# kdexd/probnmn-clevr

Hardware: AMD Instinct MI355X
Metric: CLEVR questions/sec (joint_training step) (higher is better)
Workload: dtype f32; 1 GPU; joint_training_ours.yml (NMN + seq2seq + REINFORCE), global batch 1024 = 1024 questions per GPU x 1 (BASELINE configs[3]), 14x14x1024 features, half of the batch with program supervision, fwd+bwd+[all-reduce]+clamp+Adam; global_batch=1024, per_gpu_batch=1024, parallelism=dp1

## Files before the change

### probnmn-clevr_amd/csrc/gemm.hip

```cpp
#include <hip/hip_runtime.h>
#include <stdint.h>

#include <type_traits>

#include "../../include/probnmn_hip.h"
#include "global_ptr.h"
#include "lds_optin.h"

namespace {

typedef float f32x16 __attribute__((ext_vector_type(16)));
using pnmn::as_global;
using pnmn::gfloat;

constexpr int TM = 128, TN = 128, TK = 32;
constexpr int OP_FLOATS = TM * TK;
using lchar = __attribute__((address_space(3))) char;
using gchar = __attribute__((address_space(1))) char;

struct Batch {
    pnmn_gemm_desc d[PNMN_GEMM_MAX];
    int first[PNMN_GEMM_MAX + 1];
    int n;
};

template <bool KC>
__device__ __forceinline__ void load_tile(const gfloat* base, int64_t ld, int row0, int k0, int rows, int K, bool vec, int tid,
                                          f32x4 (&r)[4], int shift_t, const gfloat* h0, int64_t ld_h0) {
#pragma unroll
    for (int j = 0; j < 4; ++j) {
        const int p = tid + 256 * j;
        f32x4 v = f32x4{0.f, 0.f, 0.f, 0.f};
        if (KC) {
            const int row = row0 + (p >> 3), k = k0 + 4 * (p & 7);
            if (row < rows && k < K) {
                const gfloat* src = base + (int64_t)row * ld + k;
                if (vec && k + 3 < K) {
                    v = pnmn::load4(src);
                } else {
#pragma unroll
                    for (int e = 0; e < 4; ++e)
                        if (k + e < K) v[e] = src[e];
                }
            }
        } else {
            const int k = k0 + (p >> 5), row = row0 + 4 * (p & 31);
            if (k < K && row < rows) {
                const gfloat* src;
                bool zero = false;
                if (shift_t > 0) {
                    const int b = k / shift_t;
                    if (k - b * shift_t == 0) {
                        zero = h0 == nullptr;
                        src = h0 + (int64_t)b * ld_h0 + row;
                    } else {
                        src = base + (int64_t)(k - 1) * ld + row;
                    }
                } else {
                    src = base + (int64_t)k * ld + row;
                }
                if (!zero) {
                    if (vec && row + 3 < rows) {
                        v = pnmn::load4(src);
                    } else {
#pragma unroll
                        for (int e = 0; e < 4; ++e)
                            if (row + e < rows) v[e] = src[e];
                    }
                }
            }
        }
        r[j] = v;
    }
}

__device__ __forceinline__ void load_tile_shift(const gfloat* base, int64_t ld, int col0, int k0, int tid, f32x4 (&r)[4], int shift_t,
                                                float rcp_t, const gfloat* h0, int64_t ld_h0) {
#pragma unroll
    for (int j = 0; j < 4; ++j) {
        const int k = k0 + (tid >> 5) + 8 * j, col = col0 + 4 * (tid & 31);
        const int b = (int)(((float)k + 0.5f) * rcp_t);
        const bool first = k == b * shift_t;
        const gfloat* prev = base + (int64_t)(k - 1) * ld + col;
        const gfloat* init = h0 ? h0 + (int64_t)b * ld_h0 + col : base + col;
        f32x4 v = pnmn::load4(first ? init : prev);
        if (first && !h0) v = f32x4{0.f, 0.f, 0.f, 0.f};
        r[j] = v;
    }
}

template <bool KC>
__device__ __forceinline__ void store_tile(float* lds, int tid, const f32x4 (&r)[4]) {
#pragma unroll
    for (int j = 0; j < 4; ++j) {
        const int p = tid + 256 * j;
        if (KC) {
            const int row = p >> 3;
            *reinterpret_cast<f32x4*>(lds + row * TK + 4 * ((p & 7) ^ ((row >> 1) & 7))) = r[j];
        } else {
            *reinterpret_cast<f32x4*>(lds + (p >> 5) * TM + 4 * (p & 31)) = r[j];
        }
    }
}

template <bool KC>
__device__ __forceinline__ f32x4 frag(const float* lds, int row, int q, int h) {
    if (KC) return *reinterpret_cast<const f32x4*>(lds + row * TK + 4 * ((2 * q + h) ^ ((row >> 1) & 7)));
    const float* p = lds + (8 * q + 4 * h) * TM + row;
    return f32x4{p[0], p[TM], p[2 * TM], p[3 * TM]};
}

template <bool KC>
struct Direct {
    const gchar* base;
    uint32_t v0, v1;
    int64_t piece, step;
    uint32_t off;

    __device__ __forceinline__ void start(const gfloat* origin, int64_t ld, int row0, int k0, int tid) {
        const int wave = __builtin_amdgcn_readfirstlane(tid >> 6), lane = tid & 63;
        const uint64_t o64 = (uint64_t)(uintptr_t)origin;
        const gchar* o = (const gchar*)(((uint64_t)(uint32_t)__builtin_amdgcn_readfirstlane((int)(o64 >> 32)) << 32) |
                                        (uint32_t)__builtin_amdgcn_readfirstlane((int)(uint32_t)o64));
        if (KC) {
            const int c = (lane & 7) ^ (lane >> 4);
            base = o + ((int64_t)(row0 + 32 * wave) * ld + k0) * 4;
            v0 = (uint32_t)((lane >> 3) * ld) * 4u + 16u * c, v1 = (uint32_t)((lane >> 3) * ld) * 4u + 16u * (c ^ 4);
            piece = 32 * ld, step = 4 * TK, off = (uint32_t)wave * 32u * 128u;
        } else {
            base = o + ((int64_t)(k0 + 8 * wave) * ld + row0) * 4;
            v0 = v1 = (uint32_t)((lane >> 5) * ld) * 4u + 16u * (lane & 31);
            piece = 8 * ld, step = 4 * (int64_t)TK * ld, off = (uint32_t)wave * 8u * 512u;
        }
    }
    __device__ __forceinline__ void issue(float* tile) {
        const uint32_t dst = __builtin_amdgcn_readfirstlane((uint32_t)(uintptr_t)((lchar*)tile)) + off;
#pragma unroll
        for (int j = 0; j < 4; ++j) {
            const uint64_t src = (uint64_t)(uintptr_t)(base + j * piece);
            asm volatile("s_mov_b32 m0, %2\n\ts_nop 0\n\tglobal_load_lds_dwordx4 %0, %1"
                         :
                         : "v"(KC && (j & 1) ? v1 : v0), "s"(src), "s"(dst + 1024u * j)
                         : "memory");
        }
        base += step;
    }
};

template <bool AKC, bool BKC>
__device__ __forceinline__ void mac_tile(const float* ca, const float* cb, int wm, int wn, int i, int h, f32x16 (&acc)[2][2], bool want_cs,
                                         float (&cs)[2]) {
#pragma unroll
    for (int q = 0; q < 4; ++q) {
        f32x4 a[2], b[2];
#pragma unroll
        for (int t = 0; t < 2; ++t) {
            a[t] = frag<AKC>(ca, 64 * wm + 32 * t + i, q, h);
            b[t] = frag<BKC>(cb, 64 * wn + 32 * t + i, q, h);
        }
        if (!AKC && want_cs) {
#pragma unroll
            for (int t = 0; t < 2; ++t) cs[t] += (a[t][0] + a[t][1]) + (a[t][2] + a[t][3]);
        }
#pragma unroll
        for (int s = 0; s < 4; ++s)
#pragma unroll
            for (int mt = 0; mt < 2; ++mt)
#pragma unroll
                for (int nt = 0; nt < 2; ++nt)
                    acc[mt][nt] = __builtin_amdgcn_mfma_f32_32x32x2f32(a[mt][s], b[nt][s], acc[mt][nt], 0, 0, 0);
    }
}

template <bool AKC, bool BKC>
__device__ __forceinline__ void contract(const pnmn_gemm_desc& d, int m0, int n0, int kbeg, int kend, float* lds, f32x16 (&acc)[2][2],
                                         bool want_cs, float (&cs)[2]) {
    const int tid = threadIdx.x, wave = tid >> 6, lane = tid & 63, i = lane & 31, h = lane >> 5;
    const int wm = wave >> 1, wn = wave & 1;
    const gfloat* A = as_global(d.a);
    const gfloat* Bm = as_global(d.b);
    const gfloat* h0 = as_global(d.shift_h0);
    const bool avec = (d.lda & 3) == 0 && ((uintptr_t)d.a & 15) == 0;
    const bool bvec = (d.ldb & 3) == 0 && ((uintptr_t)d.b & 15) == 0 && (d.shift_t == 0 || d.shift_h0 == nullptr ||
                                                                       ((d.ld_h0 & 3) == 0 && ((uintptr_t)d.shift_h0 & 15) == 0));
    float* la = lds;
    float* lb = lds + 2 * OP_FLOATS;
    const bool adir = avec && m0 + TM <= d.M, bdir = bvec && n0 + TN <= d.N && (BKC || d.shift_t == 0);
    const int kfull = kbeg + (kend - kbeg) / TK * TK;
    const float rcp_t = d.shift_t > 0 ? 1.f / (float)d.shift_t : 0.f;
    Direct<AKC> da;
    Direct<BKC> db;
    da.start(A, d.lda, m0, kbeg, tid);
    db.start(Bm, d.ldb, n0, kbeg, tid);
    auto loop = [&](auto ad_tag, auto bd_tag, int lo, int hi) {
        constexpr bool AD = decltype(ad_tag)::value, BD = decltype(bd_tag)::value;
        f32x4 ra[4], rb[4];
        auto fetch = [&](int k0, int st) {
            if constexpr (AD)
                da.issue(la + st * OP_FLOATS);
            else
                load_tile<AKC>(A, d.lda, m0, k0, d.M, kend, avec, tid, ra, 0, nullptr, 0);
            if constexpr (BD)
                db.issue(lb + st * OP_FLOATS);
            else if constexpr (AD && !BKC)
                load_tile_shift(Bm, d.ldb, n0, k0, tid, rb, d.shift_t, rcp_t, h0, d.ld_h0);
            else
                load_tile<BKC>(Bm, d.ldb, n0, k0, d.N, kend, bvec, tid, rb, BKC ? 0 : d.shift_t, h0, d.ld_h0);
        };
        auto commit = [&](int st) {
            if constexpr (!AD) store_tile<AKC>(la + st * OP_FLOATS, tid, ra);
            if constexpr (!BD) store_tile<BKC>(lb + st * OP_FLOATS, tid, rb);
        };
        if (lo >= hi) return;
        fetch(lo, 0);
        commit(0);
        asm volatile("s_waitcnt vmcnt(0)" ::: "memory");
        __syncthreads();
        int cur = 0;
        for (int k0 = lo; k0 < hi; k0 += TK) {
            const bool more = k0 + TK < hi;
            if (more) fetch(k0 + TK, cur ^ 1);
            const float* ca = la + cur * OP_FLOATS;
            const float* cb = lb + cur * OP_FLOATS;
            mac_tile<AKC, BKC>(ca, cb, wm, wn, i, h, acc, want_cs, cs);
            if (more) commit(cur ^ 1);
            asm volatile("s_waitcnt vmcnt(0)" ::: "memory");
            __syncthreads();
            cur ^= 1;
        }
    };
    using yes = std::true_type;
    using no = std::false_type;
    if (adir && bdir) {
        loop(yes{}, yes{}, kbeg, kfull);
        loop(no{}, no{}, kfull, kend);
    } else if (!BKC && adir && bvec && d.shift_t > 0 && n0 + TN <= d.N && kend <= (1 << 21)) {
        if constexpr (!BKC) {
            loop(yes{}, no{}, kbeg, kfull);
            loop(no{}, no{}, kfull, kend);
        }
    } else {
        loop(no{}, no{}, kbeg, kend);
    }
}

using gint2 = __attribute__((address_space(1))) int2;

__device__ __forceinline__ void load_rows(const gint2* list, int k0, int kend, int tid, int2 (&e)[4]) {
#pragma unroll
    for (int j = 0; j < 4; ++j) {
        const int k = k0 + (tid >> 5) + 8 * j;
        const gint2* q = list + (k < kend ? k : kend - 1);
        e[j].x = q->x, e[j].y = q->y;
    }
}

__device__ __forceinline__ void load_tile_rows(const gfloat* base, int64_t ld, int col0, int k0, int cols, int kend, bool vec, int tid,
                                               const int2 (&e)[4], f32x4 (&r)[4], bool shifted, const gfloat* h0, int64_t ld_h0) {
#pragma unroll
    for (int j = 0; j < 4; ++j) {
        const int k = k0 + (tid >> 5) + 8 * j, col = col0 + 4 * (tid & 31);
        f32x4 v = f32x4{0.f, 0.f, 0.f, 0.f};
        if (k < kend && col < cols) {
            const int row = shifted ? e[j].y : e[j].x;
            const bool first = row < 0;
            const gfloat* src = first ? (h0 ? h0 + (int64_t)(~row) * ld_h0 + col : base + col) : base + (int64_t)row * ld + col;
            if (vec && col + 3 < cols) {
                v = pnmn::load4(src);
            } else {
#pragma unroll
                for (int c = 0; c < 4; ++c)
                    if (col + c < cols) v[c] = src[c];
            }
            if (first && !h0) v = f32x4{0.f, 0.f, 0.f, 0.f};
        }
        r[j] = v;
    }
}

struct DirectRows {
    const gchar* origin;
    int64_t ld;
    uint32_t lane, off;

    __device__ __forceinline__ void start(const gfloat* base, int64_t ld_floats, int col0, int tid) {
        origin = (const gchar*)(base + col0), ld = 4 * ld_floats;
        lane = 16u * (tid & 31), off = (uint32_t)__builtin_amdgcn_readfirstlane(tid >> 6) * 1024u;
    }
    __device__ __forceinline__ void issue(float* tile, const int2 (&e)[4]) {
        const uint32_t dst = __builtin_amdgcn_readfirstlane((uint32_t)(uintptr_t)((lchar*)tile)) + off;
#pragma unroll
        for (int j = 0; j < 4; ++j) {
            const gchar* src = origin + (int64_t)e[j].x * ld + lane;
            asm volatile("s_mov_b32 m0, %1\n\ts_nop 0\n\tglobal_load_lds_dwordx4 %0, off" : : "v"(src), "s"(dst + 4096u * j) : "memory");
        }
    }
};

__device__ __forceinline__ void contract_rows(const pnmn_gemm_desc& d, const gint2* list, int m0, int n0, int kbeg, int kend, float* lds,
                                              f32x16 (&acc)[2][2], bool want_cs, float (&cs)[2]) {
    const int tid = threadIdx.x, wave = tid >> 6, lane = tid & 63, i = lane & 31, h = lane >> 5;
    const int wm = wave >> 1, wn = wave & 1;
    const gfloat* A = as_global(d.a);
    const gfloat* Bm = as_global(d.b);
    const gfloat* h0 = as_global(d.shift_h0);
    const bool shifted = d.shift_t > 0;
    const bool avec = (d.lda & 3) == 0 && ((uintptr_t)d.a & 15) == 0;
    const bool bvec = (d.ldb & 3) == 0 && ((uintptr_t)d.b & 15) == 0 &&
                      (!shifted || d.shift_h0 == nullptr || ((d.ld_h0 & 3) == 0 && ((uintptr_t)d.shift_h0 & 15) == 0));
    float* la = lds;
    float* lb = lds + 2 * OP_FLOATS;
    const bool adir = avec && m0 + TM <= d.M, bdir = bvec && n0 + TN <= d.N && !shifted;
    const int kfull = kbeg + (kend - kbeg) / TK * TK;
    DirectRows da, db;
    da.start(A, d.lda, m0, tid);
    db.start(Bm, d.ldb, n0, tid);
    auto loop = [&](auto ad_tag, auto bd_tag, int lo, int hi) {
        constexpr bool AD = decltype(ad_tag)::value, BD = decltype(bd_tag)::value;
        f32x4 ra[4], rb[4];
        int2 e[4];
        auto fetch = [&](int k0, int st) {
            if constexpr (AD)
                da.issue(la + st * OP_FLOATS, e);
            else
                load_tile_rows(A, d.lda, m0, k0, d.M, kend, avec, tid, e, ra, false, nullptr, 0);
            if constexpr (BD)
                db.issue(lb + st * OP_FLOATS, e);
            else
                load_tile_rows(Bm, d.ldb, n0, k0, d.N, kend, bvec, tid, e, rb, shifted, h0, d.ld_h0);
        };
        auto commit = [&](int st) {
            if constexpr (!AD) store_tile<false>(la + st * OP_FLOATS, tid, ra);
            if constexpr (!BD) store_tile<false>(lb + st * OP_FLOATS, tid, rb);
        };
        if (lo >= hi) return;
        load_rows(list, lo, kend, tid, e);
        fetch(lo, 0);
        load_rows(list, lo + TK, kend, tid, e);
        commit(0);
        asm volatile("s_waitcnt vmcnt(0)" ::: "memory");
        __syncthreads();
        int cur = 0;
        for (int k0 = lo; k0 < hi; k0 += TK) {
            const bool more = k0 + TK < hi;
            if (more) {
                fetch(k0 + TK, cur ^ 1);
                load_rows(list, k0 + 2 * TK, kend, tid, e);
            }
            mac_tile<false, false>(la + cur * OP_FLOATS, lb + cur * OP_FLOATS, wm, wn, i, h, acc, want_cs, cs);
            if (more) commit(cur ^ 1);
            asm volatile("s_waitcnt vmcnt(0)" ::: "memory");
            __syncthreads();
            cur ^= 1;
        }
    };
    using yes = std::true_type;
    using no = std::false_type;
    if (adir && bdir) {
        loop(yes{}, yes{}, kbeg, kfull);
        loop(no{}, no{}, kfull, kend);
    } else if (adir) {
        loop(yes{}, no{}, kbeg, kfull);
        loop(no{}, no{}, kfull, kend);
    } else {
        loop(no{}, no{}, kbeg, kend);
    }
}

struct Lists {
    const int2* rows[PNMN_GEMM_MAX];
    const int32_t* count[PNMN_GEMM_MAX];
};

template <bool LIST>
__global__ __launch_bounds__(256) __attribute__((amdgpu_waves_per_eu(2, 2))) void gemm_kernel(const Batch batch, const Lists lists) {
    extern __shared__ __attribute__((aligned(16))) float lds[];
    for (int unit = blockIdx.x; unit < batch.first[batch.n]; unit += gridDim.x) {
    int pi = 0;
    while (pi + 1 < batch.n && unit >= batch.first[pi + 1]) ++pi;
    const pnmn_gemm_desc d = batch.d[pi];
    const int local = unit - batch.first[pi];
    const int tiles_n = (d.N + TN - 1) / TN, tiles_m = (d.M + TM - 1) / TM;
    const int split = d.split_k > 1 ? d.split_k : 1;
    const int chunk = local % split, tile = local / split;
    const int tm = tile / tiles_n, tn = tile % tiles_n;
    const int m0 = tm * TM, n0 = tn * TN;
    int K = d.K;
    const gint2* list = nullptr;
    if constexpr (LIST) {
        list = (const gint2*)lists.rows[pi];
        if (list) {
            const int count = __builtin_amdgcn_readfirstlane(*(const __attribute__((address_space(1))) int32_t*)lists.count[pi]);
            K = count < 0 ? 0 : (count < d.K ? count : d.K);
        }
    }
    const int ktiles = (K + TK - 1) / TK;
    const int per = ktiles / split, extra = ktiles % split;
    const int kt0 = chunk * per + (chunk < extra ? chunk : extra);
    const int kt1 = kt0 + per + (chunk < extra ? 1 : 0);
    const int kbeg = kt0 * TK, kend = kt1 * TK < K ? kt1 * TK : K;

    f32x16 acc[2][2];
#pragma unroll
    for (int mt = 0; mt < 2; ++mt)
#pragma unroll
        for (int nt = 0; nt < 2; ++nt)
#pragma unroll
            for (int r = 0; r < 16; ++r) acc[mt][nt][r] = 0.f;
    const bool akc = !(d.flags & PNMN_GEMM_A_TRANSPOSED), bkc = (d.flags & PNMN_GEMM_B_TRANSPOSED) != 0;
    const bool want_cs = d.colsum != nullptr && !akc && tn == 0 && ((threadIdx.x >> 6) & 1) == 0;
    const bool tile_cs = d.colsum != nullptr && !akc && tn == 0;
    float cs[2] = {0.f, 0.f};
    if (LIST && list) {
        if (kbeg < kend) contract_rows(d, list, m0, n0, kbeg, kend, lds, acc, want_cs, cs);
    } else if (kbeg < kend) {
        if (akc && bkc)
            contract<true, true>(d, m0, n0, kbeg, kend, lds, acc, false, cs);
        else if (akc)
            contract<true, false>(d, m0, n0, kbeg, kend, lds, acc, false, cs);
        else if (bkc)
            contract<false, true>(d, m0, n0, kbeg, kend, lds, acc, want_cs, cs);
        else
            contract<false, false>(d, m0, n0, kbeg, kend, lds, acc, want_cs, cs);
    }

    int tid = threadIdx.x, m0e = m0, n0e = n0;
    asm volatile("" : "+v"(tid), "+s"(m0e), "+s"(n0e));
    const int wave = tid >> 6, lane = tid & 63, i = lane & 31, h = lane >> 5;
    const int wm = wave >> 1, wn = wave & 1;
    if (tile_cs) {
        if (want_cs) {
#pragma unroll
            for (int t = 0; t < 2; ++t) lds[h * TM + 64 * wm + 32 * t + i] = cs[t];
        }
        __syncthreads();
        if (tid < TM) {
            const float t = lds[tid] + lds[TM + tid];
            if (split > 1) {
                as_global(d.workspace)[(size_t)tiles_m * tiles_n * split * (TM * TN) + ((size_t)tm * split + chunk) * TM + tid] = t;
            } else if (m0e + tid < d.M) {
                d.colsum[m0e + tid] = t;
                if (d.colsum2) d.colsum2[m0e + tid] = t;
            }
        }
        __syncthreads();
    }
    if (split > 1) {
        gfloat* ws = as_global(d.workspace) + ((size_t)tile * split + chunk) * (TM * TN);
#pragma unroll
        for (int mt = 0; mt < 2; ++mt)
#pragma unroll
            for (int nt = 0; nt < 2; ++nt)
#pragma unroll
                for (int r = 0; r < 16; ++r)
                    ws[(64 * wm + 32 * mt + 8 * (r >> 2) + 4 * h + (r & 3)) * TN + 64 * wn + 32 * nt + i] = acc[mt][nt][r];
        continue;
    }
    gfloat* C = as_global(d.c);
    const gfloat* bias = as_global(d.bias);
    const bool accumulate = (d.flags & PNMN_GEMM_ACCUMULATE) != 0;
#pragma unroll
    for (int nt = 0; nt < 2; ++nt) {
        const int col = n0e + 64 * wn + 32 * nt + i;
        if (col >= d.N) continue;
        const float bv = d.bias ? bias[col] : 0.f;
#pragma unroll
        for (int mt = 0; mt < 2; ++mt)
#pragma unroll
            for (int r = 0; r < 16; ++r) {
                const int row = m0e + 64 * wm + 32 * mt + 8 * (r >> 2) + 4 * h + (r & 3);
                if (row < d.M) {
                    gfloat* dst = C + (int64_t)row * d.ldc + col;
                    float v = acc[mt][nt][r] + bv;
                    if (accumulate) v += *dst;
                    *dst = v;
                }
            }
    }
    }
}

__global__ __launch_bounds__(256) void gemm_reduce_kernel(const Batch batch) {
    int pi = 0;
    while (pi + 1 < batch.n && (int)blockIdx.x >= batch.first[pi + 1]) ++pi;
    const pnmn_gemm_desc d = batch.d[pi];
    const int local = blockIdx.x - batch.first[pi];
    const int tiles_n = (d.N + TN - 1) / TN;
    const int quarter = local & 3, tile = local >> 2;
    const int m0 = (tile / tiles_n) * TM + 32 * quarter, n0 = (tile % tiles_n) * TN;
    const int split = d.split_k, tid = threadIdx.x;
    const gfloat* wt = as_global(d.workspace) + (size_t)tile * split * (TM * TN) + quarter * (32 * TN);
    f32x4 sum[4];
#pragma unroll
    for (int j = 0; j < 4; ++j) sum[j] = f32x4{0.f, 0.f, 0.f, 0.f};
    for (int c = 0; c < split; ++c) {
        const gfloat* wc = wt + (size_t)c * (TM * TN);
        f32x4 v[4];
#pragma unroll
        for (int j = 0; j < 4; ++j) v[j] = pnmn::load4(wc + 4 * (tid + 256 * j));
#pragma unroll
        for (int j = 0; j < 4; ++j) sum[j] += v[j];
    }
    if (d.colsum && (d.flags & PNMN_GEMM_A_TRANSPOSED) && quarter == 0 && tile % tiles_n == 0 && tid < TM) {
        const int tiles_m = (d.M + TM - 1) / TM, tm = tile / tiles_n;
        const gfloat* wc = as_global(d.workspace) + (size_t)tiles_m * tiles_n * split * (TM * TN) + (size_t)tm * split * TM + tid;
        float t = 0.f;
        for (int c = 0; c < split; ++c) t += wc[(size_t)c * TM];
        if (tm * TM + tid < d.M) {
            d.colsum[tm * TM + tid] = t;
            if (d.colsum2) d.colsum2[tm * TM + tid] = t;
        }
    }
    gfloat* C = as_global(d.c);
    const gfloat* bias = as_global(d.bias);
    const bool accumulate = (d.flags & PNMN_GEMM_ACCUMULATE) != 0;
    const bool cvec = (d.ldc & 3) == 0 && ((uintptr_t)d.c & 15) == 0;
#pragma unroll
    for (int j = 0; j < 4; ++j) {
        const int p = tid + 256 * j, row = m0 + (p >> 5), col = n0 + 4 * (p & 31);
        if (row >= d.M || col >= d.N) continue;
        gfloat* dst = C + (int64_t)row * d.ldc + col;
        f32x4 v = sum[j];
        if (cvec && col + 3 < d.N) {
            if (d.bias) {
#pragma unroll
                for (int e = 0; e < 4; ++e) v[e] += bias[col + e];
            }
            if (accumulate) v += pnmn::load4(dst);
            pnmn::store4(dst, v);
        } else {
#pragma unroll
            for (int e = 0; e < 4; ++e)
                if (col + e < d.N) {
                    float x = v[e] + (d.bias ? bias[col + e] : 0.f);
                    if (accumulate) x += dst[e];
                    dst[e] = x;
                }
        }
    }
}

__global__ __launch_bounds__(256) void colsum_kernel(const float* __restrict__ x, int64_t ld, int R, int C, float* __restrict__ partial,
                                                     int* __restrict__ counter, float* __restrict__ out, float* __restrict__ out2,
                                                     int accumulate, int vec) {
    __shared__ int last_flag;
    __shared__ float red[4][256];
    const int tx = threadIdx.x & 63, ty = threadIdx.x >> 6;
    const int c0 = blockIdx.x * 256 + 4 * tx;
    const int slices = gridDim.y, s = blockIdx.y;
    const int per = (R + slices - 1) / slices;
    const int r0 = s * per, r1 = min(R, r0 + per);
    f32x4 acc[4] = {f32x4{0.f, 0.f, 0.f, 0.f}, f32x4{0.f, 0.f, 0.f, 0.f}, f32x4{0.f, 0.f, 0.f, 0.f}, f32x4{0.f, 0.f, 0.f, 0.f}};
    if (c0 < C) {
        if (vec && c0 + 3 < C) {
            int r = r0 + ty;
            for (; r + 12 < r1; r += 16) {
#pragma unroll
                for (int e = 0; e < 4; ++e) acc[e] += *reinterpret_cast<const f32x4*>(x + (int64_t)(r + 4 * e) * ld + c0);
            }
            for (; r < r1; r += 4) acc[0] += *reinterpret_cast<const f32x4*>(x + (int64_t)r * ld + c0);
        } else {
            for (int r = r0 + ty; r < r1; r += 4)
#pragma unroll
                for (int k = 0; k < 4; ++k)
                    if (c0 + k < C) acc[0][k] += x[(int64_t)r * ld + c0 + k];
        }
    }
    const f32x4 t = (acc[0] + acc[1]) + (acc[2] + acc[3]);
#pragma unroll
    for (int k = 0; k < 4; ++k) red[ty][4 * tx + k] = t[k];
    __syncthreads();
    const int c = blockIdx.x * 256 + threadIdx.x;
    if (c < C) partial[(size_t)s * C + c] = (red[0][threadIdx.x] + red[1][threadIdx.x]) + (red[2][threadIdx.x] + red[3][threadIdx.x]);
    __threadfence();
    __syncthreads();
    if (threadIdx.x == 0) {
        const int old = atomicAdd(counter + blockIdx.x, 1);
        last_flag = old == slices - 1;
        if (last_flag) counter[blockIdx.x] = 0;
    }
    __syncthreads();
    if (!last_flag || c >= C) return;
    __threadfence();
    float total = 0.f;
    for (int k = 0; k < slices; ++k) total += __builtin_nontemporal_load(partial + (size_t)k * C + c);
    if (accumulate) total += out[c];
    out[c] = total;
    if (out2) out2[c] = total;
}

}

extern "C" int64_t pnmn_gemm_workspace_bytes(int M, int N, int split_k) {
    if (split_k <= 1) return 0;
    const int64_t tiles_m = (M + TM - 1) / TM, tiles = tiles_m * ((N + TN - 1) / TN);
    return (tiles * split_k * (TM * TN) + tiles_m * split_k * TM) * (int64_t)sizeof(float);
}

extern "C" int pnmn_gemm_split_k(int M, int N, int K, int cus) {
    const int64_t tiles = (int64_t)((M + TM - 1) / TM) * ((N + TN - 1) / TN);
    const int ktiles = (K + TK - 1) / TK;
    if (cus <= 0) cus = 256;
    int64_t want = (2 * (int64_t)cus + tiles - 1) / tiles;
    if (tiles >= cus) want = 1;
    const int most = ktiles / 4 > 0 ? ktiles / 4 : 1;
    if (want > most) want = most;
    if (want > 64) want = 64;
    return want < 1 ? 1 : (int)want;
}

namespace {
int launch(const pnmn_gemm_desc* descs, int n, const int32_t* const* rows, const int32_t* const* count, int max_workgroups,
           void* stream) {
    if (n <= 0) return 0;
    if (!descs || n > PNMN_GEMM_MAX) return PNMN_EINVAL;
    Batch b;
    Lists l = {};
    bool listed = false;
    int blocks = 0, live = 0;
    for (int k = 0; k < n; ++k) {
        const pnmn_gemm_desc& d = descs[k];
        if (d.M <= 0 || d.N <= 0) continue;
        if (!d.a || !d.b || !d.c || d.K < 0) return PNMN_EINVAL;
        if (d.split_k > 1 && !d.workspace) return PNMN_EINVAL;
        if (d.shift_t > 0 && (d.flags & PNMN_GEMM_B_TRANSPOSED)) return PNMN_ESHAPE;
        if (d.colsum && !(d.flags & PNMN_GEMM_A_TRANSPOSED)) return PNMN_ESHAPE;
        l.rows[live] = nullptr, l.count[live] = nullptr;
        if (rows && rows[k]) {
            if ((d.flags & (PNMN_GEMM_A_TRANSPOSED | PNMN_GEMM_B_TRANSPOSED)) != PNMN_GEMM_A_TRANSPOSED) return PNMN_ESHAPE;
            if (!count || !count[k]) return PNMN_EINVAL;
            l.rows[live] = reinterpret_cast<const int2*>(rows[k]), l.count[live] = count[k];
            listed = true;
        }
        b.d[live] = d;
        b.first[live] = blocks;
        const int tiles = ((d.M + TM - 1) / TM) * ((d.N + TN - 1) / TN);
        blocks += tiles * (d.split_k > 1 ? d.split_k : 1);
        ++live;
    }
    if (!live) return 0;
    b.first[live] = blocks;
    b.n = live;
    constexpr size_t lds = (size_t)4 * OP_FLOATS * sizeof(float);
    static std::atomic<uint64_t> cfg{0}, cfg_rows{0};
    const int grid = (max_workgroups > 0 && max_workgroups < blocks) ? max_workgroups : blocks;
    if (listed) {
        if (const int e = pnmn::opt_in_lds(reinterpret_cast<const void*>(gemm_kernel<true>), lds, cfg_rows)) return e;
        hipLaunchKernelGGL(gemm_kernel<true>, dim3(grid), dim3(256), lds, static_cast<hipStream_t>(stream), b, l);
    } else {
        if (const int e = pnmn::opt_in_lds(reinterpret_cast<const void*>(gemm_kernel<false>), lds, cfg)) return e;
        hipLaunchKernelGGL(gemm_kernel<false>, dim3(grid), dim3(256), lds, static_cast<hipStream_t>(stream), b, l);
    }
    Batch r;
    int rblocks = 0, rlive = 0;
    for (int k = 0; k < live; ++k) {
        if (b.d[k].split_k <= 1) continue;
        r.d[rlive] = b.d[k];
        r.first[rlive] = rblocks;
        rblocks += 4 * ((b.d[k].M + TM - 1) / TM) * ((b.d[k].N + TN - 1) / TN);
        ++rlive;
    }
    if (rlive) {
        r.first[rlive] = rblocks;
        r.n = rlive;
        hipLaunchKernelGGL(gemm_reduce_kernel, dim3(rblocks), dim3(256), 0, static_cast<hipStream_t>(stream), r);
    }
    return (int)hipGetLastError();
}
}

extern "C" int pnmn_gemm(const pnmn_gemm_desc* descs, int n, void* stream) { return launch(descs, n, nullptr, nullptr, 0, stream); }

extern "C" int pnmn_gemm_cus(const pnmn_gemm_desc* descs, int n, int max_workgroups, void* stream) {
    return launch(descs, n, nullptr, nullptr, max_workgroups, stream);
}

extern "C" int pnmn_gemm_rows(const pnmn_gemm_desc* descs, int n, const int32_t* const* rows, const int32_t* const* count,
                              int max_workgroups, void* stream) {
    return launch(descs, n, rows, count, max_workgroups, stream);
}

extern "C" int64_t pnmn_colsum_workspace_bytes(int R, int C) {
    (void)R;
    return (int64_t)128 * C * sizeof(float) + (int64_t)((C + 255) / 256) * sizeof(int);
}

extern "C" int pnmn_colsum(const float* x, int64_t ld, int R, int C, float* out, float* out2, int accumulate, void* workspace,
                           void* stream) {
    if (C <= 0) return 0;
    if (!out || !workspace || (R > 0 && !x)) return PNMN_EINVAL;
    int slices = (R + 63) / 64;
    if (slices > 128) slices = 128;
    if (slices < 1) slices = 1;
    float* partial = static_cast<float*>(workspace);
    int* counter = reinterpret_cast<int*>(partial + (size_t)128 * C);
    const int vec = (ld & 3) == 0 && ((uintptr_t)x & 15) == 0;
    hipLaunchKernelGGL(colsum_kernel, dim3((C + 255) / 256, slices), dim3(256), 0, static_cast<hipStream_t>(stream), x, ld, R, C,
                       partial, counter, out, out2, accumulate, vec);
    return (int)hipGetLastError();
}
```

Baseline: 40250 questions/s.

## Extend direct global-to-LDS loads to edge tiles and cap grid for tail waves

Direct global_load_lds paths now also cover partial edge tiles. Out-of-range rows and columns are clamped to the last valid one, so edge tiles no longer fall back to register-staged loads. Per-piece vector offsets are precomputed so issue uses a single scalar base. Separately, when K-lengths across batched GEMMs are similar, the grid is capped at twice the CU count if the last wave would be partly empty, so the kernel's persistent loop balances work. Risks include reading clamped duplicate data into unused tile rows, and 32-bit offset overflow, which a leading-dimension bound guards against.

```diff
diff --git a/probnmn-clevr_amd/csrc/gemm.hip b/probnmn-clevr_amd/csrc/gemm.hip
--- a/probnmn-clevr_amd/csrc/gemm.hip
+++ b/probnmn-clevr_amd/csrc/gemm.hip
@@ -1,6 +1,7 @@
 #include <hip/hip_runtime.h>
 #include <stdint.h>
 
+#include <algorithm>
 #include <type_traits>
 
 #include "../../include/probnmn_hip.h"
@@ -113,39 +114,47 @@
 template <bool KC>
 struct Direct {
     const gchar* base;
-    uint32_t v0, v1;
-    int64_t piece, step;
+    uint32_t v[4];
+    int64_t step;
     uint32_t off;
 
-    __device__ __forceinline__ void start(const gfloat* origin, int64_t ld, int row0, int k0, int tid) {
+    __device__ __forceinline__ void start(const gfloat* origin, int64_t ld, int row0, int k0, int rows, int tid) {
         const int wave = __builtin_amdgcn_readfirstlane(tid >> 6), lane = tid & 63;
         const uint64_t o64 = (uint64_t)(uintptr_t)origin;
         const gchar* o = (const gchar*)(((uint64_t)(uint32_t)__builtin_amdgcn_readfirstlane((int)(o64 >> 32)) << 32) |
                                         (uint32_t)__builtin_amdgcn_readfirstlane((int)(uint32_t)o64));
+        const uint32_t ld32 = (uint32_t)ld;
         if (KC) {
             const int c = (lane & 7) ^ (lane >> 4);
-            base = o + ((int64_t)(row0 + 32 * wave) * ld + k0) * 4;
-            v0 = (uint32_t)((lane >> 3) * ld) * 4u + 16u * c, v1 = (uint32_t)((lane >> 3) * ld) * 4u + 16u * (c ^ 4);
-            piece = 32 * ld, step = 4 * TK, off = (uint32_t)wave * 32u * 128u;
+            const int last = rows - 1, r0 = row0 + 32 * wave, rb = r0 < last ? r0 : last;
+            base = o + ((int64_t)rb * ld + k0) * 4;
+#pragma unroll
+            for (int j = 0; j < 4; ++j) {
+                const int r = r0 + 8 * j + (lane >> 3);
+                v[j] = (uint32_t)((r < last ? r : last) - rb) * ld32 * 4u + 16u * ((j & 1) ? (c ^ 4) : c);
+            }
+            step = 4 * TK, off = (uint32_t)wave * 32u * 128u;
         } else {
-            base = o + ((int64_t)(k0 + 8 * wave) * ld + row0) * 4;
-            v0 = v1 = (uint32_t)((lane >> 5) * ld) * 4u + 16u * (lane & 31);
-            piece = 8 * ld, step = 4 * (int64_t)TK * ld, off = (uint32_t)wave * 8u * 512u;
+            const int col = row0 + 4 * (lane & 31), cl = col < rows - 4 ? col : rows - 4;
+            base = o + ((int64_t)(k0 + 8 * wave) * ld) * 4;
+#pragma unroll
+            for (int j = 0; j < 4; ++j) v[j] = ((uint32_t)(2 * j + (lane >> 5)) * ld32 + (uint32_t)cl) * 4u;
+            step = 4 * (int64_t)TK * ld, off = (uint32_t)wave * 8u * 512u;
         }
     }
     __device__ __forceinline__ void issue(float* tile) {
         const uint32_t dst = __builtin_amdgcn_readfirstlane((uint32_t)(uintptr_t)((lchar*)tile)) + off;
-#pragma unroll
-        for (int j = 0; j < 4; ++j) {
-            const uint64_t src = (uint64_t)(uintptr_t)(base + j * piece);
-            asm volatile("s_mov_b32 m0, %2\n\ts_nop 0\n\tglobal_load_lds_dwordx4 %0, %1"
-                         :
-                         : "v"(KC && (j & 1) ? v1 : v0), "s"(src), "s"(dst + 1024u * j)
-                         : "memory");
-        }
+        const uint64_t src = (uint64_t)(uintptr_t)base;
+#pragma unroll
+        for (int j = 0; j < 4; ++j)
+            asm volatile("s_mov_b32 m0, %2\n\ts_nop 0\n\tglobal_load_lds_dwordx4 %0, %1" : : "v"(v[j]), "s"(src), "s"(dst + 1024u * j) : "memory");
         base += step;
     }
 };
+
+__device__ __forceinline__ bool direct_ok(const float* ptr, int64_t ld, bool kc, int row0, int rows) {
+    return (ld & 3) == 0 && ld < (1 << 24) && ((uintptr_t)ptr & 15) == 0 && (row0 + TM <= rows || kc || (rows & 3) == 0);
+}
 
 template <bool AKC, bool BKC>
 __device__ __forceinline__ void mac_tile(const float* ca, const float* cb, int wm, int wn, int i, int h, f32x16 (&acc)[2][2], bool want_cs,
@@ -185,13 +194,13 @@
                                                                        ((d.ld_h0 & 3) == 0 && ((uintptr_t)d.shift_h0 & 15) == 0));
     float* la = lds;
     float* lb = lds + 2 * OP_FLOATS;
-    const bool adir = avec && m0 + TM <= d.M, bdir = bvec && n0 + TN <= d.N && (BKC || d.shift_t == 0);
+    const bool adir = direct_ok(d.a, d.lda, AKC, m0, d.M), bdir = direct_ok(d.b, d.ldb, BKC, n0, d.N) && (BKC || d.shift_t == 0);
     const int kfull = kbeg + (kend - kbeg) / TK * TK;
     const float rcp_t = d.shift_t > 0 ? 1.f / (float)d.shift_t : 0.f;
     Direct<AKC> da;
     Direct<BKC> db;
-    da.start(A, d.lda, m0, kbeg, tid);
-    db.start(Bm, d.ldb, n0, kbeg, tid);
+    da.start(A, d.lda, m0, kbeg, d.M, tid);
+    db.start(Bm, d.ldb, n0, kbeg, d.N, tid);
     auto loop = [&](auto ad_tag, auto bd_tag, int lo, int hi) {
         constexpr bool AD = decltype(ad_tag)::value, BD = decltype(bd_tag)::value;
         f32x4 ra[4], rb[4];
@@ -283,9 +292,10 @@
     int64_t ld;
     uint32_t lane, off;
 
-    __device__ __forceinline__ void start(const gfloat* base, int64_t ld_floats, int col0, int tid) {
-        origin = (const gchar*)(base + col0), ld = 4 * ld_floats;
-        lane = 16u * (tid & 31), off = (uint32_t)__builtin_amdgcn_readfirstlane(tid >> 6) * 1024u;
+    __device__ __forceinline__ void start(const gfloat* base, int64_t ld_floats, int col0, int cols, int tid) {
+        const int col = col0 + 4 * (tid & 31);
+        origin = (const gchar*)base, ld = 4 * ld_floats;
+        lane = 4u * (uint32_t)(col < cols - 4 ? col : cols - 4), off = (uint32_t)__builtin_amdgcn_readfirstlane(tid >> 6) * 1024u;
     }
     __device__ __forceinline__ void issue(float* tile, const int2 (&e)[4]) {
         const uint32_t dst = __builtin_amdgcn_readfirstlane((uint32_t)(uintptr_t)((lchar*)tile)) + off;
@@ -310,11 +320,11 @@
                       (!shifted || d.shift_h0 == nullptr || ((d.ld_h0 & 3) == 0 && ((uintptr_t)d.shift_h0 & 15) == 0));
     float* la = lds;
     float* lb = lds + 2 * OP_FLOATS;
-    const bool adir = avec && m0 + TM <= d.M, bdir = bvec && n0 + TN <= d.N && !shifted;
+    const bool adir = direct_ok(d.a, d.lda, false, m0, d.M), bdir = direct_ok(d.b, d.ldb, false, n0, d.N) && !shifted;
     const int kfull = kbeg + (kend - kbeg) / TK * TK;
     DirectRows da, db;
-    da.start(A, d.lda, m0, tid);
-    db.start(Bm, d.ldb, n0, tid);
+    da.start(A, d.lda, m0, d.M, tid);
+    db.start(Bm, d.ldb, n0, d.N, tid);
     auto loop = [&](auto ad_tag, auto bd_tag, int lo, int hi) {
         constexpr bool AD = decltype(ad_tag)::value, BD = decltype(bd_tag)::value;
         f32x4 ra[4], rb[4];
@@ -610,6 +620,22 @@
 }
 
 namespace {
+int compute_units(int* cus) {
+    static std::atomic<int> known[64];
+    int dev = 0;
+    hipError_t e = hipGetDevice(&dev);
+    if (e != hipSuccess) return (int)e;
+    int n = known[dev & 63].load(std::memory_order_acquire);
+    if (n <= 0) {
+        e = hipDeviceGetAttribute(&n, hipDeviceAttributeMultiprocessorCount, dev);
+        if (e != hipSuccess) return (int)e;
+        if (n <= 0) n = 256;
+        known[dev & 63].store(n, std::memory_order_release);
+    }
+    *cus = n;
+    return 0;
+}
+
 int launch(const pnmn_gemm_desc* descs, int n, const int32_t* const* rows, const int32_t* const* count, int max_workgroups,
            void* stream) {
     if (n <= 0) return 0;
@@ -643,7 +669,22 @@
     b.n = live;
     constexpr size_t lds = (size_t)4 * OP_FLOATS * sizeof(float);
     static std::atomic<uint64_t> cfg{0}, cfg_rows{0};
-    const int grid = (max_workgroups > 0 && max_workgroups < blocks) ? max_workgroups : blocks;
+    int slots = max_workgroups;
+    if (slots <= 0) {
+        int longest = 0, shortest = INT32_MAX;
+        for (int k = 0; k < live; ++k) {
+            const int ktiles = (b.d[k].K + TK - 1) / TK, split = b.d[k].split_k > 1 ? b.d[k].split_k : 1;
+            longest = std::max(longest, (ktiles + split - 1) / split), shortest = std::min(shortest, ktiles / split);
+        }
+        slots = blocks;
+        if (!listed && 4 * (int64_t)longest <= 5 * (int64_t)shortest) {
+            int cus = 0;
+            if (const int e = compute_units(&cus)) return e;
+            const int r = blocks % (2 * cus);
+            if (blocks > 2 * cus && r > 0 && r <= cus) slots = 2 * cus;
+        }
+    }
+    const int grid = slots < blocks ? slots : blocks;
     if (listed) {
         if (const int e = pnmn::opt_in_lds(reinterpret_cast<const void*>(gemm_kernel<true>), lds, cfg_rows)) return e;
         hipLaunchKernelGGL(gemm_kernel<true>, dim3(grid), dim3(256), lds, static_cast<hipStream_t>(stream), b, l);
```

Result: slower. 27930 questions/s (-30.6%).
